# IvanPopov/video-flow-ml

Hardware: AMD Instinct MI355X
Metric: flow-fields/sec @1080p seq5 MOF_sintel (higher is better)
Workload: dtype mixed (per-layer MFMA count, f32 accumulate): {"corr": 1, "update_block.encoder.convf1": 1, "update_block.encoder.convf2": 1, "update_block.gru.convq1.iter": "2a", "update_block.gru.convzr1.iter": 1, "update_block.gru.convzr2.iter": 1, "update_block.mask.0": 1, "update_block.mask.2": 1, "update_bloc

## Files before the change

### video-flow-ml_amd/vfml/csrc/conv_gemm_split.hip

```cpp
#include "conv_split_common.h"

namespace {

template <int BN, int WM, int WN, bool BIGC, bool IN16, int NM = 3>
__global__ __launch_bounds__(WM * WN * 64, 2) void conv_gemm_split_kernel(const SplitArgs a) {
  constexpr bool ALO = NM == 3 || NM == 2, BLO = NM == 3 || NM == 4;
  constexpr int NT = WM * WN * 64;
  constexpr int LR = NT / 4;
  constexpr int TM = BM / (WM * 32);
  constexpr int TN = BN / (WN * 32);
  constexpr int AU = BM / LR;
  constexpr int BU = BN / LR;
  constexpr int BUN = BU > 0 ? BU : 1;
  constexpr int RSA = BM + 2;
  constexpr int RSB = BN + 2;
  constexpr int SA = KG * RSA;
  constexpr int SB = KG * RSB;
  constexpr int LDC = BN + 4;

  extern __shared__ __attribute__((aligned(16))) char smem_raw[];
  h16x8* sAh = reinterpret_cast<h16x8*>(smem_raw);
  h16x8* sAl = sAh + 2 * SA;
  h16x8* sBh = sAl + 2 * SA;
  h16x8* sBl = sBh + 2 * SB;
// ... 1444 lines not shown
  const bool tilebase = in16 && !two && d->kh == 1 && d->kw == 1 && d->stride == 1 && d->pad_h == 0 && d->pad_w == 0 &&
                        (int64_t)256 * d->ld0 * 4 < (1ll << 31);
  if (!tilebase) {
    const int64_t px = (int64_t)d->n * d->h * d->w + (int64_t)(d->pad_h + 1) * d->w + d->pad_w;
    VFML_REQUIRE(px * d->ld0 * 4 < (1ll << 30) && (!two || px * d->ld1 * 4 < (1ll << 30)),
                 "vfml_conv2d_split: a source spans >= 1 GiB");
  }
  {
    VFML_REQUIRE(bhi ? (int64_t)d->cout * kp * 2 <= 0x7ffffff0ll : ((int64_t)d->cout + 128) * kp * 2 < (1ll << 30),
                 "vfml_conv2d_split: weight planes too large");
  }
  if (d->epilogue == VFML_EPI_GRU_ZR || d->epilogue == VFML_EPI_TANH_RELU)
    VFML_REQUIRE(d->split > 0 && d->split < d->cout && d->split % 4 == 0,
                 "vfml_conv2d_split: split=%d must be a multiple of 4 inside (0, cout)", d->split);
  if (d->epilogue == VFML_EPI_GRU_ZR || d->epilogue == VFML_EPI_ADD_AUX)
    VFML_REQUIRE(d->aux0, "vfml_conv2d_split: this epilogue needs aux0");
  if (d->epilogue == VFML_EPI_GRU_Q) VFML_REQUIRE(d->aux0 && d->aux1, "vfml_conv2d_split: GRU_Q needs aux0 and aux1");
  VFML_REQUIRE(d->epilogue >= VFML_EPI_NONE && d->epilogue <= VFML_EPI_ADD_AUX, "vfml_conv2d_split: bad epilogue");

  a.wbase = nullptr; a.whi_off = a.wlo_off = a.bytesb = 0; a.korder = k_order; a.direct = 0; a.fastk = 0; a.abias = 0; a.src1_delta = 0; a.out_t = nullptr; a.ld_out_t = 0; a.cswap = 0; a.bhi = 0;
  a.stats_part = d->stats_part;
  a.ksplit = 1; a.out_k1 = nullptr; a.out_t_k1 = nullptr;
  a.resident = 0; a.res_nc = 0; a.res_cl = 0;
  a.nm = (d->flags & VFML_CONV_MFMA1) ? 1 : (d->flags & VFML_CONV_MFMA2A) ? (bhi ? 1 : 4) : ((d->flags & VFML_CONV_MFMA2) || bhi) ? 2 : 3;
  a.pointwise = d->kh == 1 && d->kw == 1 && d->stride == 1 && d->pad_h == 0 && d->pad_w == 0;
  const float* base = (two && d->in1 < d->in0) ? d->in1 : d->in0;
  const int64_t e0 = (d->in0 - base) + ((int64_t)d->n * d->h * d->w - 1) * d->ld0 + d->c0;
  const int64_t e1 = two ? (d->in1 - base) + ((int64_t)d->n * d->h * d->w - 1) * d->ld1 + d->c1 : 0;
  VFML_REQUIRE(tilebase || (e0 > e1 ? e0 : e1) * 4 < (1ll << 31),
               "vfml_conv2d_split: in0 and in1 must be slices of one buffer (< 2 GiB apart)");
  a.in0 = base; a.in1 = base;
  a.d0off = (int)(d->in0 - base); a.d1off = two ? (int)(d->in1 - base) : 0;
  const bool fits_one = (e0 > e1 ? e0 : e1) * 4 < (1ll << 31) && (int64_t)d->n * d->h * d->w * d->ld0 * 4 < (1ll << 30);
  a.bytes0 = fits_one ? (int)((e0 > e1 ? e0 : e1) * 4) : 0;
  a.tilebase = 0;
  a.proj_w = nullptr; a.proj_lo_off = a.proj_bytes = a.proj_n = a.proj_kp = 0; a.proj_inv = 1.f; a.proj_out = nullptr; a.ld_proj = 0;
  a.whi = (const _Float16*)w_hi; a.wlo = (const _Float16*)w_lo; a.bias = d->bias;
  a.aux0 = d->aux0; a.aux1 = d->aux1; a.out = d->out;
  a.addend = d->addend; a.ld_addend = d->ld_addend;
  a.addend_ind = d->addend_ind;
  VFML_REQUIRE(!d->addend_ind || (d->addend && (reinterpret_cast<uintptr_t>(d->addend_ind) & 7u) == 0),
               "vfml_conv2d_split: addend_ind goes with an addend of the same shape and alignment (what the call validates) and is 8-byte aligned");
  a.c0 = d->c0; a.ld0 = d->ld0; a.c1 = d->c1; a.ld1 = two ? d->ld1 : d->ld0; a.ctot = d->c0 + d->c1;
  a.H = d->h; a.W = d->w; a.ho = ho; a.wo = wo;
  a.kh = d->kh; a.kw = d->kw; a.stride = d->stride; a.pad_h = d->pad_h; a.pad_w = d->pad_w;
  a.M = (int)M64; a.K = K; a.Kp = kp; a.cout = d->cout;
  a.bytesw = (int)((int64_t)d->cout * kp * 2);
// ... 78 lines not shown
    VFML_REQUIRE(a.fastk && (a.nm == 3 || a.nm == 4) && d->cout % 128 == 0,
                 "vfml_conv2d_split: proj_out needs the uniform-step loader (channel-block weight order, whole 32-channel "
                 "blocks), the full split product or VFML_CONV_MFMA2A (which then holds for the projection too) and "
                 "cout %% 128 == 0");
    VFML_REQUIRE(d->proj_hi && d->proj_lo && d->proj_n > 0 && d->proj_n <= 48 && d->proj_n % 4 == 0 && d->proj_kp >= d->cout &&
                     d->proj_kp % 8 == 0 && d->ld_proj >= d->proj_n && d->ld_proj % 4 == 0 && vfml_aligned16(d->proj_out) &&
                     vfml_aligned16(d->proj_hi) && vfml_aligned16(d->proj_lo) && d->proj_scale > 0.f,
                 "vfml_conv2d_split: proj_hi / proj_lo [proj_n <= 48, %% 4 == 0][proj_kp >= cout] f16 planes, ld_proj >= proj_n, "
                 "16-byte alignment");
    const char* ph2 = (const char*)d->proj_hi;
    const char* pl2 = (const char*)d->proj_lo;
    const int64_t plane = (int64_t)d->proj_n * d->proj_kp * 2;
    VFML_REQUIRE(pl2 >= ph2 && (pl2 - ph2) + plane < (1ll << 30), "vfml_conv2d_split: proj_lo must follow proj_hi within 1 GiB");
    a.proj_w = ph2; a.proj_lo_off = (int)(pl2 - ph2); a.proj_bytes = (int)((pl2 - ph2) + plane);
    a.proj_n = d->proj_n; a.proj_kp = d->proj_kp; a.proj_inv = 1.0f / d->proj_scale;
    a.proj_out = d->proj_out; a.ld_proj = d->ld_proj;
  }
  return 0;
}

static int dma_tile_env() {
  const char* tile_env = getenv("VFML_DMA_TILE");
  if (!tile_env) return 0;
  int tm = 2, tn = 2, wm = 2, wn = 2;
  sscanf(tile_env, "%d,%d,%d,%d", &tm, &tn, &wm, &wn);
  return tm * 1000 + tn * 100 + wm * 10 + wn;
}

static int split_prepare(const vfml_conv_desc* d, const void* w_hi, const void* w_lo, int kp, float w_scale, int in_fmt, int out_fmt,
                         int aux_fmt, int k_order, int forced_tile, SplitArgs& a, SplitPlan& plan, const SplitVariant*& row) {
  if (const int rc = split_fill(d, w_hi, w_lo, kp, w_scale, in_fmt, out_fmt, aux_fmt, k_order, a)) return rc;
  if (const int rc = vfml_detail::plan_split(a, in_fmt == VFML_FMT_S16, d->flags, forced_tile, &plan)) return rc;
  a.nm = plan.nm;
  a.fastk = plan.fastk;
  a.resident = plan.resident ? 1 : 0;
  if (!plan.fastk) a.abias = 0;
  row = plan.family == vfml_detail::SPLIT_TAPX ? vfml_detail::tapx_variant(plan)
        : plan.family == vfml_detail::SPLIT_DMA ? vfml_detail::find_variant(DMA_VARIANTS, sizeof(DMA_VARIANTS) / sizeof(DMA_VARIANTS[0]), plan)
                                                : vfml_detail::find_variant(REG_VARIANTS, sizeof(REG_VARIANTS) / sizeof(REG_VARIANTS[0]), plan);
  if (!row) {
    char name[160];
    vfml_detail::variant_name(plan, name, sizeof(name));
    vfml_set_error("vfml_conv2d_split: no such variant: %s", name);
    return 1;
  }
  return 0;
}

extern "C" int vfml_conv2d_split(const vfml_conv_desc* d, const void* w_hi, const void* w_lo, int kp, float w_scale,
                                 int in_fmt, int out_fmt, int aux_fmt, int k_order, void* stream) {
  SplitArgs a;
  SplitPlan plan;
  const SplitVariant* row;
  if (const int rc = split_prepare(d, w_hi, w_lo, kp, w_scale, in_fmt, out_fmt, aux_fmt, k_order, dma_tile_env(), a, plan, row)) return rc;
  hipStream_t s = reinterpret_cast<hipStream_t>(stream);
  const int rc = row->launch(a, s);
  if (rc || !plan.add_rows) return rc;
  const int64_t quads = (int64_t)a.M * (d->cout / 4);
// ... 31 lines not shown
```

### video-flow-ml_amd/vfml/csrc/conv_gemm_tapx.hip

```cpp
#include "conv_split_common.h"

#ifndef VFML_TAPX_HOOKS
#define TAPX_HOOK_ENTRY()
#define TAPX_HOOK_KLOOP_BEGIN()
#define TAPX_HOOK_STEP_BEGIN(st)
#define TAPX_HOOK_STAMP(k)
#define TAPX_HOOK_STEP_END()
#define TAPX_HOOK_KLOOP_END(nsteps)
#define TAPX_HOOK_EXIT()
#endif

namespace {

template <int TM, int TN, int WM, int WN, int NM>
__global__ __launch_bounds__(256, 2) void conv_gemm_tapx_kernel(const SplitArgs a) {
  constexpr bool H64 = NM == 5;
  constexpr bool BHI = NM == 2 || NM == 1 || H64;
  constexpr bool AHI = NM == 4 || NM == 1 || H64;
  constexpr int KSTEP = H64 ? 64 : 32;
  constexpr int NT = 256;
  static_assert(WM * WN == 4, "four waves: two workgroups per CU");
  constexpr int TBM = 32 * TM * WM, TBN = 32 * TN * WN;
  constexpr int NPA = (TBM + VFML_TAPX_KWMAX - 1 + 7) / 8;
  constexpr int NPI = (NPA + 3) / 4;
  constexpr int BP = TBN / 32;
  constexpr int ASZ = NPA * 1024, BSZ = TBN * 128;
  constexpr int BOFF = 2 * ASZ, ZOFF = BOFF + BSZ;
  constexpr int LDC = TBN + 4;
  static_assert(ZOFF % 128 == 0, "the zero cell must keep the fragment address bits 4..6 free");
  constexpr int ASLOTS = (NPI + 1) / 2;
  static_assert(NPI * 4 <= 64, "activation validity bits: 4 per piece in a register pair");
  static_assert(BP + ASLOTS <= 4 * TM * TN, "one issue slot per MFMA group");

  extern __shared__ __attribute__((aligned(16))) char smem_raw[];
  float* sC = reinterpret_cast<float*>(smem_raw);
  TAPX_HOOK_ENTRY();

  const int total = a.mtiles * a.ntiles;
  int tile;
  {
    const int xcd = blockIdx.x & 7, lw = blockIdx.x >> 3;
    const int q = total >> 3, r = total & 7;
    const int start = xcd < r ? xcd * (q + 1) : r * (q + 1) + (xcd - r) * q;
    tile = start + lw;
    if (tile >= start + q + (xcd < r ? 1 : 0)) return;
  }
  const int nt_ = tile % a.ntiles, mt_ = tile / a.ntiles;
  const int m0 = mt_ * TBM, n0 = nt_ * TBN;

  const int t = threadIdx.x;
  const int lane = t & 63;
  const int wave = __builtin_amdgcn_readfirstlane(t >> 6);
  if (t < 32) reinterpret_cast<float*>(smem_raw + ZOFF)[t] = 0.f;

  const int srow = lane >> 3;
  const int sw = (4 * wave + (lane >> 4)) & 7;
  const int pieceL = (lane & 7) ^ (H64 ? sw : swz16(sw));
  const __amdgpu_buffer_rsrc_t r0 = __builtin_amdgcn_make_buffer_rsrc(
      reinterpret_cast<char*>(const_cast<float*>(a.in0)) - a.abias, 0, a.bytes0 + a.abias, 0x00020000);
  const __amdgpu_buffer_rsrc_t rb = __builtin_amdgcn_make_buffer_rsrc(const_cast<char*>(a.wbase), 0, a.bytesb, 0x00020000);
  int vbaseA = ((m0 + 8 * wave + srow) * a.ld0 + a.d0off) * 4 + (H64 ? pieceL * 32 : (pieceL >> 1) * 32 + (pieceL & 1) * 16);
  if (AHI && !H64 && (pieceL & 1)) vbaseA |= (int)0x80000000;
  unsigned long long vmask = 0ull;
  {
    const int NH = a.M / a.W;
#pragma unroll
    for (int i = 0; i < NPI; ++i) {
      const int s = 8 * (4 * i + wave) + srow;
      const int base = m0 + s - a.pad_w;
      const int qb = base >= 0 ? base / a.W : -1;
      const int oy = qb - (qb / a.H) * a.H;
      const bool in = 4 * i + wave < NPA && s < TBM + a.kw - 1 && qb >= 0 && qb < NH;
      for (int ky = 0; ky < a.kh; ++ky) {
        const int iy = oy + ky - a.pad_h;
        if (!(in && iy >= 0 && iy < a.H)) vmask |= 1ull << (4 * i + ky);
      }
    }
  }
  int colbase[BP];
#pragma unroll
  for (int j = 0; j < BP; ++j) {
    const int col = n0 + 32 * j + 8 * wave + srow;
    if constexpr (H64)
      colbase[j] = col < a.cout ? a.whi_off + col * a.Kp * 2 + pieceL * 16 : 0x40000000;
    else
      colbase[j] = col < a.cout && !(BHI && (pieceL & 1)) ? ((pieceL & 1) ? a.wlo_off : a.whi_off) + col * a.Kp * 2 + (pieceL >> 1) * 16
                                                          : 0x40000000;
  }

  auto issue_a = [&](int i, int nbuf, int cbn, int kyn) {
    const int cl = cbn < a.c0 ? cbn : cbn - a.c0;
    const int soff = (kyn * a.W * a.ld0 + cl + i * 32 * a.ld0) * 4 + (cbn < a.c0 ? 0 : a.src1_delta);
    const int bad = (int)((unsigned)(vmask >> (4 * i + kyn)) << 31);
    dma16(r0, bad | vbaseA, soff, smem_raw + nbuf * ASZ + (4 * i + wave) * 1024);
  };
  auto issue_b = [&](int j, int stn) {
    dma16(rb, colbase[j], stn * (H64 ? 128 : 64), smem_raw + BOFF + wave * 1024 + j * 4096);
  };

  const int wm = wave / WN, wn = wave % WN;
  const int r4 = lane & 15, u4 = lane >> 4;
  const int pb16 = (H64 ? (u4 ^ ((r4 >> 1) & 7)) : ((2 * u4) ^ swz16((r4 >> 1) & 7))) * 16;
  const int boff4 = BOFF + (wn * (32 * TN) + r4) * 128 + pb16;
  constexpr int X1 = H64 ? 64 : 16;
  int oxp[2 * TM];
#pragma unroll
  for (int i = 0; i < 2 * TM; ++i) {
    const int m = m0 + wm * (32 * TM) + i * 16 + r4;
    oxp[i] = m - (m / a.W) * a.W - a.pad_w;
  }

  f32x4 acc4[2 * TM][2 * TN];
#pragma unroll
  for (int i = 0; i < 2 * TM; ++i)
#pragma unroll
    for (int j = 0; j < 2 * TN; ++j)
#pragma unroll
      for (int e = 0; e < 4; ++e) acc4[i][j][e] = 0.f;

  const int ncb = a.ctot / KSTEP;
  const int nstage = ncb * a.kh;
  const int nsteps = nstage * a.kw;

#pragma unroll
  for (int i = 0; i < NPI; ++i)
    if (4 * i + wave < NPA) issue_a(i, 0, 0, 0);
#pragma unroll
  for (int j = 0; j < BP; ++j) issue_b(j, 0);
  asm volatile("s_waitcnt vmcnt(0)" ::: "memory");
  __syncthreads();

  TAPX_HOOK_KLOOP_BEGIN();
  int st = 0;
  int cbn = 0, kyn = 0;
  for (int sg = 0; sg < nstage; ++sg) {
    const int abuf = (sg & 1) * ASZ;
    const int nbuf = (sg & 1) ^ 1;
    if (++kyn == a.kh) {
      kyn = 0;
      cbn += KSTEP;
    }
    const bool next_stage = sg + 1 < nstage;
    for (int kx = 0; kx < a.kw; ++kx, ++st) {
      const bool next_step = st + 1 < nsteps;
      TAPX_HOOK_STEP_BEGIN(st);
      h16x8 b0[2 * TN], b1[2 * TN];
#pragma unroll
      for (int j = 0; j < 2 * TN; ++j) {
        b0[j] = *reinterpret_cast<const h16x8*>(smem_raw + boff4 + j * 2048);
        if constexpr (H64 || !BHI) b1[j] = *reinterpret_cast<const h16x8*>(smem_raw + (boff4 ^ X1) + j * 2048);
      }
      const int R0 = r4 + kx;
      const int swa = (R0 >> 1) & 7;
      const int aoffk = abuf + (wm * (32 * TM) + R0) * 128 + (H64 ? (u4 ^ swa) : ((2 * u4) ^ swz16(swa))) * 16;
      auto a_addr = [&](int i) { return (unsigned)(oxp[i] + kx) < (unsigned)a.W ? aoffk + i * 2048 : ZOFF; };
      h16x8 a0, a1;
      {
        const int ad = a_addr(0);
        a0 = *reinterpret_cast<const h16x8*>(smem_raw + ad);
        if constexpr (H64 || !AHI) a1 = *reinterpret_cast<const h16x8*>(smem_raw + (ad ^ X1));
      }
      __syncthreads();
      TAPX_HOOK_STAMP(1);
      __builtin_amdgcn_sched_barrier(0);
      static_for<2 * TM>([&](auto ic) {
        constexpr int i = decltype(ic)::value;
        h16x8 n0_, n1_;
        if constexpr (i + 1 < 2 * TM) {
          const int ad = a_addr(i + 1);
          n0_ = *reinterpret_cast<const h16x8*>(smem_raw + ad);
          if constexpr (H64 || !AHI) n1_ = *reinterpret_cast<const h16x8*>(smem_raw + (ad ^ X1));
        }
        static_for<2 * TN>([&](auto jc) {
          constexpr int j = decltype(jc)::value;
          acc4[i][j] = __builtin_amdgcn_mfma_f32_16x16x32_f16(b0[j], a0, acc4[i][j], 0, 0, 0);
          if constexpr (H64) {
            acc4[i][j] = __builtin_amdgcn_mfma_f32_16x16x32_f16(b1[j], a1, acc4[i][j], 0, 0, 0);
          } else {
            if constexpr (!BHI) acc4[i][j] = __builtin_amdgcn_mfma_f32_16x16x32_f16(b1[j], a0, acc4[i][j], 0, 0, 0);
            if constexpr (!AHI) acc4[i][j] = __builtin_amdgcn_mfma_f32_16x16x32_f16(b0[j], a1, acc4[i][j], 0, 0, 0);
          }
          constexpr int g = i * (2 * TN) + j;
          if constexpr (g < BP) {
            if (next_step) issue_b(g, st + 1);
          } else if constexpr (g < BP + ASLOTS) {
            const int ia = kx + (g - BP) * a.kw;
            if (next_stage && ia < NPI && 4 * ia + wave < NPA) issue_a(ia, nbuf, cbn, kyn);
          }
          __builtin_amdgcn_sched_barrier(0);
        });
        if constexpr (i + 1 < 2 * TM) {
          a0 = n0_;
          if constexpr (H64 || !AHI) a1 = n1_;
        }
      });
      TAPX_HOOK_STAMP(2);
      asm volatile("s_waitcnt vmcnt(0)" ::: "memory");
      TAPX_HOOK_STAMP(3);
      __syncthreads();
      TAPX_HOOK_STEP_END();
    }
  }

  TAPX_HOOK_KLOOP_END(nsteps);
#pragma unroll
  for (int i = 0; i < TM; ++i) {
    if (i) lds_barrier();
    static_for<2>([&](auto tc) {
      constexpr int t2 = decltype(tc)::value;
      static_for<2 * TN>([&](auto jc) {
        constexpr int j = decltype(jc)::value;
        f32x4 v = {0.f, 0.f, 0.f, 0.f};
        static_for<TM>([&](auto ii) { if (decltype(ii)::value == i) v = acc4[2 * decltype(ii)::value + t2][j]; });
        *reinterpret_cast<f32x4*>(&sC[(wm * 32 + t2 * 16 + r4) * LDC + wn * (32 * TN) + j * 16 + 4 * u4]) = v;
      });
    });
    lds_barrier();
    if (!epilogue_rows_fast<TBN, NT>(a, sC, m0, n0, t, WM * 32, 32 * TM, i * 32))
      epilogue_rows<TBN, NT>(a, sC, m0, n0, t, WM * 32, 32 * TM, i * 32);
    if (a.stats_part) {
      for (int p = t; p < TBN * WM; p += NT) {
        const int ch = p % TBN, wb = p / TBN;
        const int g0 = m0 + wb * (32 * TM) + i * 32;
        if (n0 + ch < a.cout && g0 < a.M) {
          const float b = a.bias ? a.bias[n0 + ch] : 0.f;
          double s1 = 0.0, s2 = 0.0;
          for (int rr = 0; rr < 32; ++rr) {
            if (g0 + rr >= a.M) break;
            const double v = (double)((sC[(wb * 32 + rr) * LDC + ch] * a.w_inv + b) * a.out_scale);
            s1 += v;
            s2 += v * v;
          }
          double* o = a.stats_part + ((int64_t)(g0 >> 5) * a.cout + n0 + ch) * 2;
          o[0] = s1;
          o[1] = s2;
        }
      }
    }
  }
  TAPX_HOOK_EXIT();
}

template <int TM, int TN, int WM, int WN, int NM>
int launch_tapx_k(SplitArgs& a, hipStream_t s) {
  constexpr int TBM = 32 * TM * WM, TBN = 32 * TN * WN;
  constexpr int NPA = (TBM + VFML_TAPX_KWMAX - 1 + 7) / 8;
  constexpr size_t stage = 2 * (size_t)NPA * 1024 + (size_t)TBN * 128 + 128;
  constexpr size_t slab = (size_t)WM * 32 * (TBN + 4) * 4;
  constexpr size_t lds = stage > slab ? stage : slab;
  static_assert(lds <= 80 * 1024, "two workgroups per CU");
  a.mtiles = (a.M + TBM - 1) / TBM;
  a.ntiles = (a.cout + TBN - 1) / TBN;
  if (const int rc = vfml_lds_cap(reinterpret_cast<const void*>(&conv_gemm_tapx_kernel<TM, TN, WM, WN, NM>), (int)lds,
                                  "vfml_conv2d_split"))
    return rc;
  hipLaunchKernelGGL((conv_gemm_tapx_kernel<TM, TN, WM, WN, NM>), dim3(a.mtiles * a.ntiles), dim3(256), lds, s, a);
  return vfml_check_launch("vfml_conv2d_split");
}

#define TAPX_ROWS(TM, TN, WM, WN) \
  {vfml_detail::tapx_plan(TM, TN, WM, WN, 3), &launch_tapx_k<TM, TN, WM, WN, 3>}, \
  {vfml_detail::tapx_plan(TM, TN, WM, WN, 5), &launch_tapx_k<TM, TN, WM, WN, 5>}
const SplitVariant TAPX_VARIANTS[] = {TAPX_ROWS(3, 2, 2, 2), TAPX_ROWS(2, 3, 2, 2), TAPX_ROWS(2, 2, 4, 1), TAPX_ROWS(2, 3, 4, 1)};
#undef TAPX_ROWS

}
// ... 10 lines not shown
```

### video-flow-ml_amd/vfml/csrc/conv_split_common.h

```cpp
#pragma once
#include <hip/hip_fp16.h>
#include <stdlib.h>
#include <utility>
#include "vfml_common.h"


namespace vfml_detail {
struct SplitArgs {
  const float* in0; const float* in1;
  const _Float16* whi; const _Float16* wlo; const float* bias;
  const float* aux0; const float* aux1; const float* addend;
  float* out;
  int c0, ld0, c1, ld1, ctot, ld_addend;
  int H, W, ho, wo;
  int kh, kw, stride, pad_h, pad_w;
  int M, K, Kp, cout;
  int d0off, d1off;
  int bytes0, bytesw;
  int ldo, ld_aux0, ld_aux1;
  int epilogue, split;
  float out_scale, w_inv;
  int mtiles, ntiles;
  int vec_ok;
  int out16, aux16;
  int out_h16;
  const char* wbase; int whi_off, wlo_off, bytesb;
  int korder;
  int direct;
  int pointwise;
  int fastk, abias, src1_delta;
  int tilebase;
  float* out_t; int ld_out_t;
  int cswap;
  int bhi;
  double* stats_part;
  int nm;
  int ksplit; float* out_k1; float* out_t_k1;
  const char* proj_w; int proj_lo_off, proj_bytes, proj_n, proj_kp; float proj_inv; float* proj_out; int ld_proj;
  const float* const* addend_ind;
  int resident, res_nc, res_cl;
};
#define VFML_RESIDENT_KMAX 256
#define VFML_RESIDENT_LDS (80 * 1024)
#define VFML_TAPX_KWMAX 5

enum SplitFamily { SPLIT_REG, SPLIT_DMA, SPLIT_TAPX };
struct SplitPlan {
  SplitFamily family;
  int bn;
  int tm, tn;
  int wm, wn;
  bool bigc, in16;
  bool persist, fastk, cswap, mf16, h16;
  int nm;
  bool add_rows;
  bool resident;
};
int plan_split(const SplitArgs& a, bool in16, int flags, int forced_tile, SplitPlan* plan);
constexpr SplitPlan reg_plan(int bn, int wm, int wn, bool bigc, bool in16, int nm) {
  return {SPLIT_REG, bn, 0, 0, wm, wn, bigc, in16, false, false, false, false, false, nm, false};
}
constexpr SplitPlan dma_plan(int tm, int tn, int wm, int wn, bool persist, bool fastk, bool cswap, int nm, bool mf16, bool h16) {
  return {SPLIT_DMA, 0, tm, tn, wm, wn, false, false, persist, fastk, cswap, mf16, h16, nm, false};
}
constexpr SplitPlan tapx_plan(int tm, int tn, int wm, int wn, int nm) {
  return {SPLIT_TAPX, 0, tm, tn, wm, wn, false, false, false, true, false, true, false, nm, false};
}
struct SplitVariant {
  SplitPlan key;
  int (*launch)(SplitArgs& a, hipStream_t s);
};
const SplitVariant* find_variant(const SplitVariant* rows, size_t n, const SplitPlan& plan);
int variant_name(const SplitPlan& key, char* buf, int len);
const SplitVariant* tapx_variant(const SplitPlan& plan);
const SplitVariant* tapx_variant_at(int index);
}
using vfml_detail::SplitArgs;
using vfml_detail::SplitPlan;
using vfml_detail::SplitVariant;
// ... 11 lines not shown

typedef _Float16 h16x8 __attribute__((ext_vector_type(8)));
typedef _Float16 h16x2 __attribute__((ext_vector_type(2)));
typedef __fp16 fp16x2 __attribute__((ext_vector_type(2)));

constexpr int BM = 128;
constexpr int BK = 32;
constexpr int KG = BK / 8;

typedef unsigned int u32x4 __attribute__((ext_vector_type(4)));
typedef unsigned int u32x2 __attribute__((ext_vector_type(2)));

__device__ __forceinline__ u32x4 bload16(__amdgpu_buffer_rsrc_t rsrc, int voff_bytes) {
  return __builtin_bit_cast(u32x4, __builtin_amdgcn_raw_buffer_load_b128(rsrc, voff_bytes, 0, 0));
}
constexpr int OOB = 0x7fffffff;

__device__ __forceinline__ float sigmoidf_(float v) { return 1.0f / (1.0f + expf(-v)); }

typedef const __attribute__((address_space(1))) float* vfml_gfptr;
typedef const __attribute__((address_space(1))) f32x4* vfml_gf4ptr;
__device__ __forceinline__ vfml_gfptr addend_of(const SplitArgs& a) {
  return (vfml_gfptr)(a.addend_ind ? *a.addend_ind : a.addend);
}

union U8 {
  h16x8 v;
  h16x2 p[4];
};

__device__ __forceinline__ void split4(const f32x4 x, U8& hi, U8& lo, int at) {
#pragma unroll
  for (int e = 0; e < 2; ++e) vfml_split2(x[2 * e], x[2 * e + 1], hi.p[at / 2 + e], lo.p[at / 2 + e]);
}

__device__ __forceinline__ float epi1(float v, int epilogue, bool lowhalf, float x0, float x1) {
  switch (epilogue) {
    case VFML_EPI_RELU: return fmaxf(v, 0.f);
    case VFML_EPI_TANH: return tanhf(v);
    case VFML_EPI_SIGMOID: return sigmoidf_(v);
    case VFML_EPI_TANH_RELU: return lowhalf ? tanhf(v) : fmaxf(v, 0.f);
    case VFML_EPI_GRU_ZR: v = sigmoidf_(v); return lowhalf ? v : v * x0;
    case VFML_EPI_GRU_Q: return (1.f - x0) * x1 + x0 * tanhf(v);
    case VFML_EPI_ADD_AUX: return x0 + v;
    default: return v;
  }
}

template <int TM, int TN, int LDC>
__device__ __forceinline__ void acc_to_lds(const f32x16 (&acc)[TM][TN], float* sC, int row0, int col0, int r, int half) {
#pragma unroll
  for (int j = 0; j < TN; ++j)
#pragma unroll
    for (int i = 0; i < TM; ++i)
#pragma unroll
      for (int e = 0; e < 16; ++e) {
        const int row = row0 + i * 32 + (e & 3) + 8 * (e >> 2) + 4 * half;
        const int col = col0 + j * 32 + r;
        sC[row * LDC + col] = acc[i][j][e];
      }
}

template <int BN, int NT>
__device__ __forceinline__ void epilogue_rows(const SplitArgs& a, const float* sC, int m0, int n0, int t,
                                              int nrows = BM, int rstride = 32, int roff = 0) {
  constexpr int LDC = BN + 4;
  constexpr int C8 = BN / 8;
  constexpr int RPP = NT / C8;
  if constexpr (NT % C8 != 0) {
    if (t >= RPP * C8) return;
  }
  const int c8 = t % C8;
  const int gcol = n0 + c8 * 8;
  if (gcol >= a.cout) return;
  const int epi = a.epilogue;
  const vfml_gfptr addend = addend_of(a);
  f32x4 bias4[2] = {{0.f, 0.f, 0.f, 0.f}, {0.f, 0.f, 0.f, 0.f}};
  if (a.bias) {
#pragma unroll
    for (int e = 0; e < 8; ++e)
      if (gcol + e < a.cout) bias4[e >> 2][e & 3] = a.bias[gcol + e];
  }
  auto aux4 = [&](const float* base, int ld, int64_t row, int col) -> f32x4 {
    f32x4 x;
    if (a.aux16) {
      const char* u = reinterpret_cast<const char*>(base + row * ld + (col & ~7)) + (col & 4) * 2;
      const h16x2 h0 = *reinterpret_cast<const h16x2*>(u), h1 = *reinterpret_cast<const h16x2*>(u + 4);
      const h16x2 l0 = *reinterpret_cast<const h16x2*>(u + 16), l1 = *reinterpret_cast<const h16x2*>(u + 20);
      x[0] = (float)h0[0] + (float)l0[0];
      x[1] = (float)h0[1] + (float)l0[1];
      x[2] = (float)h1[0] + (float)l1[0];
      x[3] = (float)h1[1] + (float)l1[1];
    } else if (a.vec_ok) {
      x = *reinterpret_cast<const f32x4*>(base + row * ld + col);
    } else {
#pragma unroll
      for (int e = 0; e < 4; ++e) x[e] = base[row * ld + col + e];
    }
    return x;
  };
  for (int row = t / C8; row < nrows; row += RPP) {
    const int grow = m0 + (row >> 5) * rstride + roff + (row & 31);
    if (grow >= a.M) continue;
#pragma unroll
    for (int q = 0; q < 2; ++q) {
      const int col = gcol + 4 * q;
      if (col >= a.cout) break;
      const bool lowhalf = col < a.split;
      const int nvalid = a.cout - col >= 4 ? 4 : a.cout - col;
      f32x4 v = *reinterpret_cast<const f32x4*>(&sC[row * LDC + c8 * 8 + 4 * q]);
      f32x4 add4 = {0.f, 0.f, 0.f, 0.f};
      if (a.addend) {
        if (nvalid == 4 && a.vec_ok) {
          add4 = *(vfml_gf4ptr)(addend + (int64_t)grow * a.ld_addend + col);
        } else {
          for (int e = 0; e < nvalid; ++e) add4[e] = addend[(int64_t)grow * a.ld_addend + col + e];
        }
      }
#pragma unroll
      for (int e = 0; e < 4; ++e) v[e] = (v[e] * a.w_inv + add4[e] + bias4[q][e]) * a.out_scale;
      f32x4 x0 = {0.f, 0.f, 0.f, 0.f}, x1 = {0.f, 0.f, 0.f, 0.f};
      if (nvalid == 4) {
        if (epi == VFML_EPI_GRU_ZR && !lowhalf) x0 = aux4(a.aux0, a.ld_aux0, grow, col - a.split);
        if (epi == VFML_EPI_GRU_Q) {
          x0 = aux4(a.aux0, a.ld_aux0, grow, col);
          x1 = aux4(a.aux1, a.ld_aux1, grow, col);
// ... 32 lines not shown
template <int EPI>
__device__ __forceinline__ void epi_unit(f32x4 (&v)[2], const f32x4 (&x0)[2], const f32x4 (&x1)[2], bool lowhalf) {
#pragma unroll
  for (int q = 0; q < 2; ++q)
#pragma unroll
    for (int e = 0; e < 4; ++e) {
      float r = v[q][e];
      if constexpr (EPI == VFML_EPI_RELU) r = fmaxf(r, 0.f);
      else if constexpr (EPI == VFML_EPI_TANH) r = tanhf(r);
      else if constexpr (EPI == VFML_EPI_SIGMOID) r = sigmoidf_(r);
      else if constexpr (EPI == VFML_EPI_GRU_ZR) { r = sigmoidf_(r); r = lowhalf ? r : r * x0[q][e]; }
      else if constexpr (EPI == VFML_EPI_GRU_Q) r = (1.f - x0[q][e]) * x1[q][e] + x0[q][e] * tanhf(r);
      v[q][e] = r;
    }
}

__device__ __forceinline__ void load_unit16(const float* base, int64_t off, f32x4 (&x)[2]) {
  const h16x8 h = *reinterpret_cast<const h16x8*>(base + off);
  const h16x8 l = *reinterpret_cast<const h16x8*>(base + off + 4);
#pragma unroll
  for (int e = 0; e < 8; ++e) x[e >> 2][e & 3] = (float)h[e] + (float)l[e];
}

template <int BN, int NT, int EPI>
__device__ __forceinline__ void epilogue_rows_fast_k(const SplitArgs& a, const float* sC, int m0, int n0, int t, int nrows,
                                                     int rstride, int roff) {
  constexpr int LDC = BN + 4;
  constexpr int C8 = BN / 8;
  constexpr int RPP = NT / C8;
  if constexpr (NT % C8 != 0) {
    if (t >= RPP * C8) return;
  }
  const int c8 = t % C8;
  const int gcol = n0 + c8 * 8;
  if (gcol >= a.cout) return;
  const bool whole = gcol + 8 <= a.cout;
  f32x4 bias4[2] = {{0.f, 0.f, 0.f, 0.f}, {0.f, 0.f, 0.f, 0.f}};
  if (a.bias) {
    bias4[0] = *reinterpret_cast<const f32x4*>(a.bias + gcol);
    if (whole) bias4[1] = *reinterpret_cast<const f32x4*>(a.bias + gcol + 4);
  }
  const bool lowhalf = gcol < a.split;
  const vfml_gfptr addend = addend_of(a);
  struct RowOps {
    f32x4 add[2], x0[2], x1[2];
  };
  auto load_row = [&](int row, RowOps& o) {
    const int grow = m0 + (row >> 5) * rstride + roff + (row & 31);
    o.add[0] = o.add[1] = f32x4{0.f, 0.f, 0.f, 0.f};
    o.x0[0] = o.x0[1] = o.x1[0] = o.x1[1] = f32x4{0.f, 0.f, 0.f, 0.f};
    if (row >= nrows || grow >= a.M) return;
    if (a.addend) {
      o.add[0] = *(vfml_gf4ptr)(addend + (int64_t)grow * a.ld_addend + gcol);
      if (whole) o.add[1] = *(vfml_gf4ptr)(addend + (int64_t)grow * a.ld_addend + gcol + 4);
    }
    if constexpr (EPI == VFML_EPI_GRU_ZR) {
      if (!lowhalf) load_unit16(a.aux0, (int64_t)grow * a.ld_aux0 + gcol - a.split, o.x0);
    }
    if constexpr (EPI == VFML_EPI_GRU_Q) {
      load_unit16(a.aux0, (int64_t)grow * a.ld_aux0 + gcol, o.x0);
      load_unit16(a.aux1, (int64_t)grow * a.ld_aux1 + gcol, o.x1);
    }
  };
  constexpr int EB = EPI == VFML_EPI_GRU_Q ? 2 : 4;
  for (int row0 = t / C8; row0 < nrows; row0 += EB * RPP) {
    RowOps ops[EB];
    static_for<EB>([&](auto bc) { load_row(row0 + decltype(bc)::value * RPP, ops[decltype(bc)::value]); });
    static_for<EB>([&](auto bc) {
      constexpr int b = decltype(bc)::value;
      const int row = row0 + b * RPP;
      const int grow = m0 + (row >> 5) * rstride + roff + (row & 31);
      if (row < nrows && grow < a.M) {
        const RowOps& cur = ops[b];
        f32x4 v[2];
        v[0] = *reinterpret_cast<const f32x4*>(&sC[row * LDC + c8 * 8]);
        v[1] = *reinterpret_cast<const f32x4*>(&sC[row * LDC + c8 * 8 + 4]);
#pragma unroll
        for (int q = 0; q < 2; ++q)
#pragma unroll
          for (int e = 0; e < 4; ++e) v[q][e] = (v[q][e] * a.w_inv + cur.add[q][e] + bias4[q][e]) * a.out_scale;
        epi_unit<EPI>(v, cur.x0, cur.x1, lowhalf);
        if (a.out16) {
          U8 hi, lo;
          split4(v[0], hi, lo, 0);
          split4(v[1], hi, lo, 4);
          float* u = a.out + (int64_t)grow * a.ldo + gcol;
          if (whole) {
            *reinterpret_cast<h16x8*>(u) = hi.v;
            *reinterpret_cast<h16x8*>(u + 4) = lo.v;
          } else {
            *reinterpret_cast<uint2*>(u) = __builtin_bit_cast(uint2, __builtin_shufflevector(hi.v, hi.v, 0, 1, 2, 3));
            *reinterpret_cast<uint2*>(u + 4) = __builtin_bit_cast(uint2, __builtin_shufflevector(lo.v, lo.v, 0, 1, 2, 3));
          }
        } else {
          float* o = a.out + (int64_t)grow * a.ldo + gcol;
// ... 78 lines not shown
    for (int j = 0; j < 3; ++j) {
      d[j] = __builtin_amdgcn_mfma_f32_16x16x32_f16(bh[j], ah, d[j], 0, 0, 0);
      d[j] = __builtin_amdgcn_mfma_f32_16x16x32_f16(bl[j], ah, d[j], 0, 0, 0);
      if constexpr (!AHI) d[j] = __builtin_amdgcn_mfma_f32_16x16x32_f16(bh[j], al, d[j], 0, 0, 0);
    }
  });
  const int srow = 16 * wave + r;
  const int grow = m0 + (srow >> 5) * rstride + roff + (srow & 31);
  if (srow < nrows && grow < a.M) {
    float* o = a.proj_out + ((int64_t)(n0 / BN) * a.M + grow) * a.ld_proj;
#pragma unroll
    for (int j = 0; j < 3; ++j) {
      const int n = 16 * j + 4 * g;
      if (n < a.proj_n) {
        f32x4 v = d[j];
#pragma unroll
        for (int e = 0; e < 4; ++e) v[e] *= a.proj_inv;
        *reinterpret_cast<f32x4*>(o + n) = v;
      }
    }
  }
}

template <int BN, int NT>
__device__ __forceinline__ bool epilogue_rows_fast(const SplitArgs& a, const float* sC, int m0, int n0, int t, int nrows,
                                                   int rstride, int roff) {
  const bool gru = a.epilogue == VFML_EPI_GRU_ZR || a.epilogue == VFML_EPI_GRU_Q;
  if (!(a.vec_ok && a.cout % 4 == 0 && (!gru || (a.aux16 && a.split % 8 == 0 && a.cout % 8 == 0)) &&
        (!a.bias || (reinterpret_cast<uintptr_t>(a.bias) & 15u) == 0) && a.epilogue != VFML_EPI_TANH_RELU &&
        a.epilogue != VFML_EPI_ADD_AUX))
    return false;
  switch (a.epilogue) {
    case VFML_EPI_NONE: epilogue_rows_fast_k<BN, NT, VFML_EPI_NONE>(a, sC, m0, n0, t, nrows, rstride, roff); return true;
    case VFML_EPI_RELU: epilogue_rows_fast_k<BN, NT, VFML_EPI_RELU>(a, sC, m0, n0, t, nrows, rstride, roff); return true;
    case VFML_EPI_GRU_ZR: epilogue_rows_fast_k<BN, NT, VFML_EPI_GRU_ZR>(a, sC, m0, n0, t, nrows, rstride, roff); return true;
    case VFML_EPI_GRU_Q: epilogue_rows_fast_k<BN, NT, VFML_EPI_GRU_Q>(a, sC, m0, n0, t, nrows, rstride, roff); return true;
    default: return false;
  }
}

typedef __attribute__((address_space(3))) void* lds_ptr_t;

__device__ __forceinline__ void dma16(__amdgpu_buffer_rsrc_t rsrc, int voff_bytes, int soff_bytes, char* lds) {
#if defined(__HIP_DEVICE_COMPILE__)
  __builtin_amdgcn_raw_ptr_buffer_load_lds(rsrc, (lds_ptr_t)lds, 16, voff_bytes, soff_bytes, 0, 0);
#endif
}

__device__ __forceinline__ constexpr int swz16(int x) { return x ^ ((((x >> 1) ^ (x >> 2)) & 1) << 1); }

}
```

### video-flow-ml_amd/vfml/csrc/conv_split_plan.hip

```cpp
#include <stdio.h>
#include "conv_split_common.h"

namespace vfml_detail {

namespace {

double reg_eff(const SplitArgs& a, int w) {
  const int nt = (a.cout + w - 1) / w;
  const int64_t wg = (int64_t)a.mtiles * nt, slots = 512;
  const int64_t rounds = (wg + slots - 1) / slots;
  return ((double)a.cout / (nt * w)) * ((double)wg / (rounds * slots)) * (w == 64 ? 0.7 : 1.0);
}

double dma_cost(const SplitArgs& a, int tbm, int tbn, double mf, double eff) {
  const double tiles = (double)((a.M + tbm - 1) / tbm) * (double)((a.cout + tbn - 1) / tbn);
  return (tiles > 512.0 ? tiles / 512.0 : 1.0) * mf / eff;
}

int tapx_cfg(const SplitArgs& a, int cfg, bool forced) {
  if (!(a.fastk && !a.direct && !a.pointwise && !a.tilebase && a.stride == 1 && a.ho == a.H && a.wo == a.W && a.kw >= 2 &&
        a.kw <= VFML_TAPX_KWMAX && a.kh <= 4 && (a.nm == 3 || a.nm == 5)))
    return 0;
  if (a.cout <= 32) return 0;
  if (forced) return (cfg == 3222 || cfg == 2322 || (cfg == 2241 && a.cout <= 64) || (cfg == 2341 && a.cout <= 96)) ? cfg : 0;
  if (a.cout <= 96) {
    const int64_t tiles = (a.M + 255) / 256, rounds = (tiles + 511) / 512;
    if (tiles * 100 < rounds * 512 * 85) return 0;
    return a.cout <= 64 ? 2241 : 2341;
  }
  return cfg == 3222 || cfg == 2322 ? cfg : 0;
}

}

int plan_split(const SplitArgs& a, bool in16, int flags, int forced_tile, SplitPlan* plan) {
  if (!in16) {
    int bn = a.cout > 64 ? 128 : (a.cout > 32 ? 64 : 32);
    if (a.cout > 64 && reg_eff(a, 64) > reg_eff(a, 128)) bn = 64;
    *plan = reg_plan(bn, bn == 32 ? 4 : 2, bn == 32 ? 1 : 2, a.ctot >= BK, false, a.nm);
    return 0;
  }

  if (a.direct) {
    VFML_REQUIRE(a.fastk || !(a.nm == 2 && a.bhi), "vfml_conv2d_split: a weight operand without lo plane needs the uniform-step GEMM form");
    const bool reduced = a.fastk && !a.cswap && (a.nm == 1 || a.nm == 2 || a.nm == 5);
    *plan = dma_plan(2, 2, 2, 2, true, a.fastk, a.cswap, reduced ? a.nm : 3, false, a.out_h16);
    plan->add_rows = a.ksplit == 2;
    plan->resident = plan->nm == 5 && plan->fastk && !plan->cswap && a.pointwise && a.ksplit == 1 && a.c1 == 0 &&
                     a.Kp <= VFML_RESIDENT_KMAX;
    return 0;
  }

  int cfg = a.cout > 32 ? 2122 : 1141;
  if (a.cout > 64) {
    const double c3222 = dma_cost(a, 192, 128, 6.0, 1.0), c2322 = dma_cost(a, 128, 192, 6.0, 1.0),
                 c2222 = dma_cost(a, 128, 128, 4.0, 0.93), c2122 = dma_cost(a, 128, 64, 2.0, 0.7);
    cfg = 3222;
    double best = c3222;
    if (c2322 < best) { best = c2322; cfg = 2322; }
    if (c2222 < best) { best = c2222; cfg = 2222; }
    if (c2122 < best) { best = c2122; cfg = 2122; }
    if (a.proj_out && cfg != 3222 && cfg != 2222) cfg = c3222 <= c2222 ? 3222 : 2222;
  }
  bool forced = false;
  if (forced_tile && a.cout > 32) {
    if (a.cout > 64 || forced_tile == 2241 || forced_tile == 2341) { cfg = forced_tile; forced = true; }
    VFML_REQUIRE(!a.proj_out || cfg == 3222 || cfg == 2222, "vfml_conv2d_split: proj_out runs on the 192 x 128 / 128 x 128 tiles (VFML_DMA_TILE)");
  }

  if (!(flags & VFML_CONV_PER_TAP) && !a.proj_out) {
    const int t = tapx_cfg(a, cfg, forced);
    if (t && (forced || a.nm == 5 || t == 2241 || t == 2341)) {
      *plan = tapx_plan(t / 1000, t / 100 % 10, t / 10 % 10, t % 10, a.nm);
      return 0;
    }
  }

  if (cfg == 2241 || cfg == 2341) cfg = 2122;
  if (cfg != 3222 && cfg != 2322 && cfg != 2122 && cfg != 1141) cfg = 2222;
  const bool fastk = a.fastk && cfg != 1141;
  VFML_REQUIRE(fastk || a.nm != 5, "vfml_conv2d_split: no 64-channel-step variant for this tile shape");
  *plan = dma_plan(cfg / 1000, cfg / 100 % 10, cfg / 10 % 10, cfg % 10, false, fastk, false, a.nm, true, false);
  return 0;
}

const SplitVariant* find_variant(const SplitVariant* rows, size_t n, const SplitPlan& p) {
  for (size_t i = 0; i < n; ++i) {
    const SplitPlan& k = rows[i].key;
    if (k.family == p.family && k.bn == p.bn && k.tm == p.tm && k.tn == p.tn && k.wm == p.wm && k.wn == p.wn && k.bigc == p.bigc &&
        k.in16 == p.in16 && k.persist == p.persist && k.fastk == p.fastk && k.cswap == p.cswap && k.mf16 == p.mf16 &&
        k.h16 == p.h16 && k.nm == p.nm)
      return &rows[i];
  }
  return nullptr;
}

// ... 15 lines not shown
```

Measured before the change: 47.21.

## Add column-walk mode to tapx conv kernel for vertical kh×1 convolutions

Adds a 'walk' variant of the tap-expanded conv GEMM kernel that handles kh×1 (vertical) convolutions by walking pixels in column-major order. Each vertical kernel then becomes a horizontal tap sweep over contiguous rows of the tile. This lets such convs use the tap-reuse tapx path instead of the per-tap DMA kernel. Output rows are remapped back to NHWC using magic-number divmod in the epilogue. It costs scattered A-row loads and output stores, and per-row index arithmetic.

```diff
diff --git a/video-flow-ml_amd/vfml/csrc/conv_gemm_split.hip b/video-flow-ml_amd/vfml/csrc/conv_gemm_split.hip
--- a/video-flow-ml_amd/vfml/csrc/conv_gemm_split.hip
+++ b/video-flow-ml_amd/vfml/csrc/conv_gemm_split.hip
@@ -1490,7 +1490,8 @@
   a.stats_part = d->stats_part;
   a.ksplit = 1; a.out_k1 = nullptr; a.out_t_k1 = nullptr;
   a.resident = 0; a.res_nc = 0; a.res_cl = 0;
-  a.nm = (d->flags & VFML_CONV_MFMA1) ? 1 : (d->flags & VFML_CONV_MFMA2A) ? (bhi ? 1 : 4) : ((d->flags & VFML_CONV_MFMA2) || bhi) ? 2 : 3;
+  a.walk_h = 0; a.walk_mh = a.walk_mw = 0;
+  a.nm =(d->flags & VFML_CONV_MFMA1) ? 1 : (d->flags & VFML_CONV_MFMA2A) ? (bhi ? 1 : 4) : ((d->flags & VFML_CONV_MFMA2) || bhi) ? 2 : 3;
   a.pointwise = d->kh == 1 && d->kw == 1 && d->stride == 1 && d->pad_h == 0 && d->pad_w == 0;
   const float* base = (two && d->in1 < d->in0) ? d->in1 : d->in0;
   const int64_t e0 = (d->in0 - base) + ((int64_t)d->n * d->h * d->w - 1) * d->ld0 + d->c0;
@@ -1615,9 +1616,9 @@
 static int dma_tile_env() {
   const char* tile_env = getenv("VFML_DMA_TILE");
   if (!tile_env) return 0;
-  int tm = 2, tn = 2, wm = 2, wn = 2;
-  sscanf(tile_env, "%d,%d,%d,%d", &tm, &tn, &wm, &wn);
-  return tm * 1000 + tn * 100 + wm * 10 + wn;
+  int tm = 2, tn = 2, wm = 2, wn = 2, walk = 0;
+  sscanf(tile_env, "%d,%d,%d,%d,%d", &tm, &tn, &wm, &wn, &walk);
+  return tm * 1000 + tn * 100 + wm * 10 + wn + (walk == 1 ? 10000 : 0);
 }
 
 static int split_prepare(const vfml_conv_desc* d, const void* w_hi, const void* w_lo, int kp, float w_scale, int in_fmt, int out_fmt,
@@ -1627,6 +1628,11 @@
   a.nm = plan.nm;
   a.fastk = plan.fastk;
   a.resident = plan.resident ? 1 : 0;
+  if (plan.walk) {
+    a.walk_h = a.H;
+    a.walk_mh = vfml_detail::walk_magic(a.H);
+    a.walk_mw = vfml_detail::walk_magic(a.W);
+  }
   if (!plan.fastk) a.abias = 0;
   row = plan.family == vfml_detail::SPLIT_TAPX ? vfml_detail::tapx_variant(plan)
         : plan.family == vfml_detail::SPLIT_DMA ? vfml_detail::find_variant(DMA_VARIANTS, sizeof(DMA_VARIANTS) / sizeof(DMA_VARIANTS[0]), plan)
diff --git a/video-flow-ml_amd/vfml/csrc/conv_gemm_tapx.hip b/video-flow-ml_amd/vfml/csrc/conv_gemm_tapx.hip
--- a/video-flow-ml_amd/vfml/csrc/conv_gemm_tapx.hip
+++ b/video-flow-ml_amd/vfml/csrc/conv_gemm_tapx.hip
@@ -12,8 +12,8 @@
 
 namespace {
 
-template <int TM, int TN, int WM, int WN, int NM>
-__global__ __launch_bounds__(256, 2) void conv_gemm_tapx_kernel(const SplitArgs a) {
+template <int TM, int TN, int WM, int WN, int NM, bool WALK>
+__device__ __forceinline__ void tapx_tile(const SplitArgs& a) {
   constexpr bool H64 = NM == 5;
   constexpr bool BHI = NM == 2 || NM == 1 || H64;
   constexpr bool AHI = NM == 4 || NM == 1 || H64;
@@ -59,10 +59,14 @@
   const __amdgpu_buffer_rsrc_t r0 = __builtin_amdgcn_make_buffer_rsrc(
       reinterpret_cast<char*>(const_cast<float*>(a.in0)) - a.abias, 0, a.bytes0 + a.abias, 0x00020000);
   const __amdgpu_buffer_rsrc_t rb = __builtin_amdgcn_make_buffer_rsrc(const_cast<char*>(a.wbase), 0, a.bytesb, 0x00020000);
-  int vbaseA = ((m0 + 8 * wave + srow) * a.ld0 + a.d0off) * 4 + (H64 ? pieceL * 32 : (pieceL >> 1) * 32 + (pieceL & 1) * 16);
-  if (AHI && !H64 && (pieceL & 1)) vbaseA |= (int)0x80000000;
+  constexpr bool walk = WALK;
+  const int kw = walk ? a.kh : a.kw, kh = walk ? 1 : a.kh;
+  const int padw = walk ? a.pad_h : a.pad_w;
+  const int L = walk ? a.H : a.W;
+  const int vlane = H64 ? pieceL * 32 : (pieceL >> 1) * 32 + (pieceL & 1) * 16;
+  int voffA[NPI];
   unsigned long long vmask = 0ull;
-  {
+  if (!walk) {
     const int NH = a.M / a.W;
 #pragma unroll
     for (int i = 0; i < NPI; ++i) {
@@ -77,6 +81,30 @@
       }
     }
   }
+  static_for<NPI>([&](auto ic) {
+    constexpr int i = decltype(ic)::value;
+    const int s = 8 * (4 * i + wave) + srow;
+    int v = ((m0 + s) * a.ld0 + a.d0off) * 4 + vlane;
+    if (walk) {
+      const int mm = m0 + s - padw;
+      const bool in = 4 * i + wave < NPA && s < TBM + kw - 1 && mm >= 0 && mm < a.M;
+      v = in ? (walk_pixel_col(a, mm) * a.ld0 + a.d0off) * 4 + a.abias + vlane : 0;
+      if (!in) vmask |= 1ull << (4 * i);
+    }
+    if (AHI && !H64 && (pieceL & 1)) v |= (int)0x80000000;
+    voffA[i] = v;
+  });
+  auto piece_off = [&](int i) __attribute__((always_inline)) {
+    int v = voffA[0];
+    static_for<NPI - 1>([&](auto kc) {
+      int w = voffA[decltype(kc)::value + 1];
+#if defined(__HIP_DEVICE_COMPILE__)
+      asm("" : "+v"(w));
+#endif
+      v = i == decltype(kc)::value + 1 ? w : v;
+    });
+    return v;
+  };
   int colbase[BP];
 #pragma unroll
   for (int j = 0; j < BP; ++j) {
@@ -88,11 +116,14 @@
                                                           : 0x40000000;
   }
 
-  auto issue_a = [&](int i, int nbuf, int cbn, int kyn) {
+  auto issue_a = [&](int i, int nbuf, int cbn, int kyn) __attribute__((always_inline)) {
     const int cl = cbn < a.c0 ? cbn : cbn - a.c0;
-    const int soff = (kyn * a.W * a.ld0 + cl + i * 32 * a.ld0) * 4 + (cbn < a.c0 ? 0 : a.src1_delta);
+    int soff = (kyn * a.W * a.ld0 + cl) * 4 + (cbn < a.c0 ? 0 : a.src1_delta);
+    int voff = voffA[0];
+    if (walk) voff = piece_off(i);
+    else soff += i * 32 * a.ld0 * 4;
     const int bad = (int)((unsigned)(vmask >> (4 * i + kyn)) << 31);
-    dma16(r0, bad | vbaseA, soff, smem_raw + nbuf * ASZ + (4 * i + wave) * 1024);
+    dma16(r0, bad | voff, soff, smem_raw + nbuf * ASZ + (4 * i + wave) * 1024);
   };
   auto issue_b = [&](int j, int stn) {
     dma16(rb, colbase[j], stn * (H64 ? 128 : 64), smem_raw + BOFF + wave * 1024 + j * 4096);
@@ -107,7 +138,7 @@
 #pragma unroll
   for (int i = 0; i < 2 * TM; ++i) {
     const int m = m0 + wm * (32 * TM) + i * 16 + r4;
-    oxp[i] = m - (m / a.W) * a.W - a.pad_w;
+    oxp[i] = m - (m / L) * L - padw;
   }
 
   f32x4 acc4[2 * TM][2 * TN];
@@ -119,8 +150,8 @@
       for (int e = 0; e < 4; ++e) acc4[i][j][e] = 0.f;
 
   const int ncb = a.ctot / KSTEP;
-  const int nstage = ncb * a.kh;
-  const int nsteps = nstage * a.kw;
+  const int nstage = ncb * kh;
+  const int nsteps = nstage * kw;
 
 #pragma unroll
   for (int i = 0; i < NPI; ++i)
@@ -136,12 +167,13 @@
   for (int sg = 0; sg < nstage; ++sg) {
     const int abuf = (sg & 1) * ASZ;
     const int nbuf = (sg & 1) ^ 1;
-    if (++kyn == a.kh) {
+    if (++kyn == kh) {
       kyn = 0;
       cbn += KSTEP;
     }
     const bool next_stage = sg + 1 < nstage;
-    for (int kx = 0; kx < a.kw; ++kx, ++st) {
+#pragma nounroll
+    for (int kx = 0; kx < kw; ++kx, ++st) {
       const bool next_step = st + 1 < nsteps;
       TAPX_HOOK_STEP_BEGIN(st);
       h16x8 b0[2 * TN], b1[2 * TN];
@@ -153,7 +185,7 @@
       const int R0 = r4 + kx;
       const int swa = (R0 >> 1) & 7;
       const int aoffk = abuf + (wm * (32 * TM) + R0) * 128 + (H64 ? (u4 ^ swa) : ((2 * u4) ^ swz16(swa))) * 16;
-      auto a_addr = [&](int i) { return (unsigned)(oxp[i] + kx) < (unsigned)a.W ? aoffk + i * 2048 : ZOFF; };
+      auto a_addr = [&](int i) { return (unsigned)(oxp[i] + kx) < (unsigned)L ? aoffk + i * 2048 : ZOFF; };
       h16x8 a0, a1;
       {
         const int ad = a_addr(0);
@@ -184,7 +216,7 @@
           if constexpr (g < BP) {
             if (next_step) issue_b(g, st + 1);
           } else if constexpr (g < BP + ASLOTS) {
-            const int ia = kx + (g - BP) * a.kw;
+            const int ia = kx + (g - BP) * kw;
             if (next_stage && ia < NPI && 4 * ia + wave < NPA) issue_a(ia, nbuf, cbn, kyn);
           }
           __builtin_amdgcn_sched_barrier(0);
@@ -216,9 +248,9 @@
       });
     });
     lds_barrier();
-    if (!epilogue_rows_fast<TBN, NT>(a, sC, m0, n0, t, WM * 32, 32 * TM, i * 32))
-      epilogue_rows<TBN, NT>(a, sC, m0, n0, t, WM * 32, 32 * TM, i * 32);
-    if (a.stats_part) {
+    if (!epilogue_rows_fast<TBN, NT, WALK>(a, sC, m0, n0, t, WM * 32, 32 * TM, i * 32))
+      epilogue_rows<TBN, NT, WALK>(a, sC, m0, n0, t, WM * 32, 32 * TM, i * 32);
+    if (!WALK && a.stats_part) {
       for (int p = t; p < TBN * WM; p += NT) {
         const int ch = p % TBN, wb = p / TBN;
         const int g0 = m0 + wb * (32 * TM) + i * 32;
@@ -242,6 +274,17 @@
 }
 
 template <int TM, int TN, int WM, int WN, int NM>
+__global__ __launch_bounds__(256, 2) void conv_gemm_tapx_kernel(const SplitArgs a) {
+  if constexpr (NM == 5 && WM == 2 && WN == 2) {
+    if (a.walk_h != 0) {
+      tapx_tile<TM, TN, WM, WN, NM, true>(a);
+      return;
+    }
+  }
+  tapx_tile<TM, TN, WM, WN, NM, false>(a);
+}
+
+template <int TM, int TN, int WM, int WN, int NM>
 int launch_tapx_k(SplitArgs& a, hipStream_t s) {
   constexpr int TBM = 32 * TM * WM, TBN = 32 * TN * WN;
   constexpr int NPA = (TBM + VFML_TAPX_KWMAX - 1 + 7) / 8;
diff --git a/video-flow-ml_amd/vfml/csrc/conv_split_common.h b/video-flow-ml_amd/vfml/csrc/conv_split_common.h
--- a/video-flow-ml_amd/vfml/csrc/conv_split_common.h
+++ b/video-flow-ml_amd/vfml/csrc/conv_split_common.h
@@ -39,7 +39,9 @@
   const char* proj_w; int proj_lo_off, proj_bytes, proj_n, proj_kp; float proj_inv; float* proj_out; int ld_proj;
   const float* const* addend_ind;
   int resident, res_nc, res_cl;
+  int walk_h; unsigned walk_mh, walk_mw;
 };
+inline unsigned walk_magic(int d) { return d > 1 ? (unsigned)((1ull << 32) / (unsigned)d) : 0xffffffffu; }
 #define VFML_RESIDENT_KMAX 256
 #define VFML_RESIDENT_LDS (80 * 1024)
 #define VFML_TAPX_KWMAX 5
@@ -55,6 +57,7 @@
   int nm;
   bool add_rows;
   bool resident;
+  bool walk;
 };
 int plan_split(const SplitArgs& a, bool in16, int flags, int forced_tile, SplitPlan* plan);
 constexpr SplitPlan reg_plan(int bn, int wm, int wn, bool bigc, bool in16, int nm) {
@@ -112,6 +115,27 @@
 typedef const __attribute__((address_space(1))) f32x4* vfml_gf4ptr;
 __device__ __forceinline__ vfml_gfptr addend_of(const SplitArgs& a) {
   return (vfml_gfptr)(a.addend_ind ? *a.addend_ind : a.addend);
+}
+
+__device__ __forceinline__ int walk_divmod(int m, int d, unsigned magic, int& rem) {
+  int q = (int)__umulhi((unsigned)m, magic);
+  rem = m - q * d;
+  if (rem >= d) {
+    ++q;
+    rem -= d;
+  }
+  return q;
+}
+__device__ __forceinline__ int walk_pixel_col(const SplitArgs& a, int m) {
+  int y, x;
+  const int c = walk_divmod(m, a.walk_h, a.walk_mh, y);
+  const int n = walk_divmod(c, a.W, a.walk_mw, x);
+  return (n * a.walk_h + y) * a.W + x;
+}
+template <bool WALK>
+__device__ __forceinline__ int walk_pixel(const SplitArgs& a, int m) {
+  if constexpr (WALK) return walk_pixel_col(a, m);
+  else return m;
 }
 
 union U8 {
@@ -151,7 +175,7 @@
       }
 }
 
-template <int BN, int NT>
+template <int BN, int NT, bool WALK = false>
 __device__ __forceinline__ void epilogue_rows(const SplitArgs& a, const float* sC, int m0, int n0, int t,
                                               int nrows = BM, int rstride = 32, int roff = 0) {
   constexpr int LDC = BN + 4;
@@ -190,8 +214,9 @@
     return x;
   };
   for (int row = t / C8; row < nrows; row += RPP) {
-    const int grow = m0 + (row >> 5) * rstride + roff + (row & 31);
-    if (grow >= a.M) continue;
+    const int trow = m0 + (row >> 5) * rstride + roff + (row & 31);
+    if (trow >= a.M) continue;
+    const int grow = walk_pixel<WALK>(a, trow);
 #pragma unroll
     for (int q = 0; q < 2; ++q) {
       const int col = gcol + 4 * q;
@@ -270,7 +295,7 @@
   for (int e = 0; e < 8; ++e) x[e >> 2][e & 3] = (float)h[e] + (float)l[e];
 }
 
-template <int BN, int NT, int EPI>
+template <int BN, int NT, int EPI, bool WALK>
 __device__ __forceinline__ void epilogue_rows_fast_k(const SplitArgs& a, const float* sC, int m0, int n0, int t, int nrows,
                                                      int rstride, int roff) {
   constexpr int LDC = BN + 4;
@@ -294,10 +319,11 @@
     f32x4 add[2], x0[2], x1[2];
   };
   auto load_row = [&](int row, RowOps& o) {
-    const int grow = m0 + (row >> 5) * rstride + roff + (row & 31);
+    const int trow = m0 + (row >> 5) * rstride + roff + (row & 31);
     o.add[0] = o.add[1] = f32x4{0.f, 0.f, 0.f, 0.f};
     o.x0[0] = o.x0[1] = o.x1[0] = o.x1[1] = f32x4{0.f, 0.f, 0.f, 0.f};
-    if (row >= nrows || grow >= a.M) return;
+    if (row >= nrows || trow >= a.M) return;
+    const int grow = walk_pixel<WALK>(a, trow);
     if (a.addend) {
       o.add[0] = *(vfml_gf4ptr)(addend + (int64_t)grow * a.ld_addend + gcol);
       if (whole) o.add[1] = *(vfml_gf4ptr)(addend + (int64_t)grow * a.ld_addend + gcol + 4);
@@ -317,8 +343,9 @@
     static_for<EB>([&](auto bc) {
       constexpr int b = decltype(bc)::value;
       const int row = row0 + b * RPP;
-      const int grow = m0 + (row >> 5) * rstride + roff + (row & 31);
-      if (row < nrows && grow < a.M) {
+      const int trow = m0 + (row >> 5) * rstride + roff + (row & 31);
+      if (row < nrows && trow < a.M) {
+        const int grow = walk_pixel<WALK>(a, trow);
         const RowOps& cur = ops[b];
         f32x4 v[2];
         v[0] = *reinterpret_cast<const f32x4*>(&sC[row * LDC + c8 * 8]);
@@ -443,7 +470,7 @@
   }
 }
 
-template <int BN, int NT>
+template <int BN, int NT, bool WALK = false>
 __device__ __forceinline__ bool epilogue_rows_fast(const SplitArgs& a, const float* sC, int m0, int n0, int t, int nrows,
                                                    int rstride, int roff) {
   const bool gru = a.epilogue == VFML_EPI_GRU_ZR || a.epilogue == VFML_EPI_GRU_Q;
@@ -452,10 +479,10 @@
         a.epilogue != VFML_EPI_ADD_AUX))
     return false;
   switch (a.epilogue) {
-    case VFML_EPI_NONE: epilogue_rows_fast_k<BN, NT, VFML_EPI_NONE>(a, sC, m0, n0, t, nrows, rstride, roff); return true;
-    case VFML_EPI_RELU: epilogue_rows_fast_k<BN, NT, VFML_EPI_RELU>(a, sC, m0, n0, t, nrows, rstride, roff); return true;
-    case VFML_EPI_GRU_ZR: epilogue_rows_fast_k<BN, NT, VFML_EPI_GRU_ZR>(a, sC, m0, n0, t, nrows, rstride, roff); return true;
-    case VFML_EPI_GRU_Q: epilogue_rows_fast_k<BN, NT, VFML_EPI_GRU_Q>(a, sC, m0, n0, t, nrows, rstride, roff); return true;
+    case VFML_EPI_NONE: epilogue_rows_fast_k<BN, NT, VFML_EPI_NONE, WALK>(a, sC, m0, n0, t, nrows, rstride, roff); return true;
+    case VFML_EPI_RELU: epilogue_rows_fast_k<BN, NT, VFML_EPI_RELU, WALK>(a, sC, m0, n0, t, nrows, rstride, roff); return true;
+    case VFML_EPI_GRU_ZR: epilogue_rows_fast_k<BN, NT, VFML_EPI_GRU_ZR, WALK>(a, sC, m0, n0, t, nrows, rstride, roff); return true;
+    case VFML_EPI_GRU_Q: epilogue_rows_fast_k<BN, NT, VFML_EPI_GRU_Q, WALK>(a, sC, m0, n0, t, nrows, rstride, roff); return true;
     default: return false;
   }
 }
diff --git a/video-flow-ml_amd/vfml/csrc/conv_split_plan.hip b/video-flow-ml_amd/vfml/csrc/conv_split_plan.hip
--- a/video-flow-ml_amd/vfml/csrc/conv_split_plan.hip
+++ b/video-flow-ml_amd/vfml/csrc/conv_split_plan.hip
@@ -29,6 +29,11 @@
     return a.cout <= 64 ? 2241 : 2341;
   }
   return cfg == 3222 || cfg == 2322 ? cfg : 0;
+}
+
+bool walk_cfg(const SplitArgs& a, int cfg) {
+  return a.fastk && !a.direct && !a.tilebase && !a.stats_part && a.stride == 1 && a.ho == a.H && a.wo == a.W && a.kw == 1 &&
+         a.pad_w == 0 && a.kh >= 2 && a.kh <= VFML_TAPX_KWMAX && a.nm == 5 && (cfg == 3222 || cfg == 2322);
 }
 
 }
@@ -63,6 +68,8 @@
     if (a.proj_out && cfg != 3222 && cfg != 2222) cfg = c3222 <= c2222 ? 3222 : 2222;
   }
   bool forced = false;
+  const bool forced_walk = forced_tile >= 10000;
+  forced_tile %= 10000;
   if (forced_tile && a.cout > 32) {
     if (a.cout > 64 || forced_tile == 2241 || forced_tile == 2341) { cfg = forced_tile; forced = true; }
     VFML_REQUIRE(!a.proj_out || cfg == 3222 || cfg == 2222, "vfml_conv2d_split: proj_out runs on the 192 x 128 / 128 x 128 tiles (VFML_DMA_TILE)");
@@ -72,6 +79,11 @@
     const int t = tapx_cfg(a, cfg, forced);
     if (t && (forced || a.nm == 5 || t == 2241 || t == 2341)) {
       *plan = tapx_plan(t / 1000, t / 100 % 10, t / 10 % 10, t % 10, a.nm);
+      return 0;
+    }
+    if (walk_cfg(a, cfg) && (!forced || forced_walk)) {
+      *plan = tapx_plan(cfg / 1000, cfg / 100 % 10, cfg / 10 % 10, cfg % 10, a.nm);
+      plan->walk = true;
       return 0;
     }
   }
```

Measured after the change: 47.42, median of 6. About the same (+0.4%).
